# cudagu/aero-gnn

Hardware: AMD Instinct MI355X
Metric: million edge-updates/sec, 1M-node/6M-edge mesh, 1->8 MI355X (higher is better)
Workload: dtype bf16; 1 GPU; BSMS-MGN 4-scale U-Net train step (fwd+MSE+bwd+allreduce+Adam), 1000000 nodes / 5996000 edges per GPU; model=BiStridedMeshGraphNet(H=128, n_hid=2, processor_size=15, stride=2, concat_trick), mode=train, global_batch=1, parallelism=dp1

## Files before the change

### aero-gnn_amd/aerognn/_lib.py

```python
from __future__ import annotations

import ctypes as C
import os

_HERE = os.path.dirname(os.path.abspath(__file__))
LIB_PATH = os.environ.get("AEROGNN_LIB") or os.path.join(_HERE, "libaerognn.so")

MAX_LIN = 8
MAX_SEG = 3
F32, BF16, F16, F64 = 0, 1, 2, 3
SEG_PLAIN, SEG_GATHER, SEG_SUM, SEG_MEAN = 0, 1, 2, 3
OPT_RESIDENT = 0

vp = C.c_void_p
i32 = C.c_int


class Seg(C.Structure):
    _fields_ = [("kind", i32), ("k", i32), ("ld", i32), ("_pad", i32),
                ("ptr", vp), ("index", vp), ("store", vp)]


ACT = {"relu": 0, "gelu": 1, "silu": 2, "tanh": 3}

# ... 44 lines not shown
                ("w_in", vp), ("w_out", vp), ("out", vp), ("dout", vp), ("gw", vp), ("s_csc", vp), ("dh", vp),
                ("dpa", vp), ("dpb", vp), ("dtx", vp), ("dw_in", vp), ("partial", vp)]


class EdgeBwdArgs(C.Structure):
    _fields_ = [("rows", i32), ("nblk", i32), ("wpk", vp * 4), ("bias", vp * 4), ("ln_g", vp), ("e", vp),
                ("proj", vp), ("src", vp), ("dst", vp), ("g", vp), ("g2", vp), ("de", vp), ("g0", vp),
                ("dw_partial", vp), ("db_partial", vp), ("ln_partial", vp), ("stamps", vp),
                ("a1", vp), ("stats", vp), ("scratch", vp), ("wtpk0", vp),
                ("xk", i32), ("xld", i32)]


class EdgeFwdArgs(C.Structure):
    _fields_ = [("rows", i32), ("nblk", i32), ("wpk", vp * 4), ("bias", vp * 4), ("ln_g", vp), ("ln_b", vp),
                ("e", vp), ("proj", vp), ("src", vp), ("dst", vp), ("out", vp), ("act", vp * 3), ("hpre", vp),
                ("stats", vp)]


class PackDesc(C.Structure):
    _fields_ = [("src", vp), ("dst", vp), ("src_dtype", i32), ("dst_dtype", i32),
                ("rows", i32), ("cols", i32), ("trans", i32), ("ld", i32),
                ("row_off", i32), ("col_off", i32), ("dst_rows", i32), ("dst_cols", i32)]


class F64Seg(C.Structure):
    _fields_ = [("a", vp), ("aidx", vp), ("lda", i32), ("k", i32), ("w", vp), ("ldw", i32), ("transw", i32)]


class F64GemmArgs(C.Structure):
    _fields_ = [("rows", i32), ("n", i32), ("nseg", i32), ("_pad", i32), ("seg", F64Seg * 3), ("bias", vp),
                ("add", vp * 2), ("add_idx", vp * 2), ("add_ld", i32 * 2), ("mask", vp), ("mask_ld", i32),
# ... 5 lines not shown
    _fields_ = [("rows", i32), ("m", i32), ("k", i32), ("_pad", i32), ("g", vp), ("ldg", i32), ("_pad1", i32),
                ("x", vp), ("ldx", i32), ("_pad2", i32), ("xidx", vp), ("dw", vp), ("ldw", i32), ("_pad3", i32),
                ("db", vp)]


_lib = None

LAUNCHES = ("agn_pack", "agn_mlp_forward", "agn_mlp_backward", "agn_reduce_partials", "agn_wgrad", "agn_wgrad_segsum", "agn_colsum",
            "agn_segment_sum", "agn_segment_sum2", "agn_gather_rows", "agn_radix_sort_u64", "agn_row_ptr", "agn_row_ptr_i64",
            "agn_iota_keys", "agn_level_index",
            "agn_exclusive_scan_i32", "agn_pool_sort_keys", "agn_pool_assign", "agn_pool_edge_candidates",
            "agn_pool_edge_sort", "agn_pool_edge_emit", "agn_bfs_distance", "agn_center_seed", "agn_maxdeg_seed",
            "agn_bistride_select", "agn_index_map", "agn_subgraph_edges", "agn_scatter_rows", "agn_wec_forward",
            "agn_wec_backward", "agn_edge_features", "agn_node_features", "agn_normalize", "agn_col_stats", "agn_collate",
            "agn_segment_max", "agn_segment_max_backward", "agn_edge_bwd_fused", "agn_encoder_bwd_fused", "agn_wgrad_reduce",
            "agn_edge_forward32",
            "agn_proj_forward", "agn_proj_backward", "agn_fourier_embed", "agn_fourier_embed_bwd")


class AeroGNNError(RuntimeError):
    pass


class _Lib:

    def __init__(self, cdll):
        self._cdll = cdll
        for name in LAUNCHES:
            if hasattr(cdll, name):
                setattr(self, name, _timed_launch(getattr(cdll, name), name[4:]))

# ... 71 lines not shown
            "agn_index_map": (i32, [vp, i32, i32, vp, vp]),
            "agn_subgraph_edges": (i32, [vp, vp, i32, vp, vp, vp, C.POINTER(i32), vp, vp]),
            "agn_scatter_rows": (i32, [i32, i32, i32, vp, vp, i32, vp, i32, vp]),
            "agn_wec_blocks": (i32, [i32]),
            "agn_edge_bwd_blocks": (i32, [i32]),
            "agn_edge_bwd_scratch_bytes": (C.c_size_t, [i32]),
            "agn_edge_features": (i32, [i32, C.c_int64, i32, vp, vp, i32, vp, vp, vp, vp, vp]),
            "agn_normalize": (i32, [i32, i32, vp, i32, vp, vp, vp, i32, i32, vp]),
            "agn_col_stats_temp_bytes": (C.c_size_t, [i32, i32]),
            "agn_col_stats": (i32, [i32, i32, vp, i32, vp, vp, C.c_float, vp, vp]),
            "agn_collate": (i32, [i32, C.c_int64, C.c_int64, vp, vp, vp, vp, vp]),
            "agn_edge_bwd_fused": (i32, [C.POINTER(EdgeBwdArgs), vp]),
            "agn_encoder_bwd_fused": (i32, [C.POINTER(EdgeBwdArgs), vp]),
            "agn_edge_fwd32_blocks": (i32, [i32]),
            "agn_edge_forward32": (i32, [C.POINTER(EdgeFwdArgs), vp]),
            "agn_debug_node32_launches": (C.c_long, []),
            "agn_debug_enc32_launches": (C.c_long, []),
            "agn_debug_dec32_launches": (C.c_long, []),
            "agn_debug_node32_bwd_launches": (C.c_long, []),
            "agn_debug_dec32_bwd_launches": (C.c_long, []),
            "agn_fault_status": (i32, [C.POINTER(i32), i32]),
            "agn_fault_status_async": (i32, [vp, vp]),
            "agn_debug_set_fault": (i32, [i32]),
            "agn_wgrad_reduce": (i32, [C.POINTER(WgradBatch), i32, vp]),
            "agn_proj_forward": (i32, [i32, vp, i32, vp, vp, vp, i32, vp]),
            "agn_proj_backward": (i32, [i32, vp, vp, i32, vp, vp, i32, vp]),
            "agn_wec_forward": (i32, [C.POINTER(WecArgs), vp]),
            "agn_wec_backward": (i32, [C.POINTER(WecArgs), vp]),
            "agn_fourier_embed": (i32, [i32, i32, i32, vp, i32, i32, i32, i32, i32, vp, i32, vp]),
            "agn_fourier_embed_bwd": (i32, [i32, i32, i32, vp, i32, i32, i32, i32, i32, vp, i32, vp, i32, vp]),
# ... 39 lines not shown
```

### aero-gnn_amd/aerognn/core.py

```python
from __future__ import annotations

import ctypes as C

import torch

from . import _lib as L
from ._lib import check, ptr


def stream():
    return C.c_void_p(torch.cuda.current_stream().cuda_stream)


PROF = None
_TIMED_DEPTH = 0


class _Timed:
    __slots__ = ("tag", "cost", "s", "on")

    def __init__(self, tag, cost):
        self.tag, self.cost = tag, cost
        self.on = False

# ... 253 lines not shown
    return (os.environ.get("AEROGNN_FUSED_EDGE_BWD", "1") != "0" and dtype == torch.bfloat16 and hidden == 128
            and nlin == 4 and has_ln and rows >= 64 * 1024)


def edge32_ok(dtype, hidden, nlin, has_ln, act=0):
    import os
    return (os.environ.get("AEROGNN_EDGE32", "1") != "0" and dtype == torch.bfloat16 and hidden == 128
            and nlin == 4 and has_ln and act == 0)


def edge_saves_ok():
    import os
    return os.environ.get("AEROGNN_EB_SAVED", "1") != "0"


def edge_forward(*, rows, wpk, bias, ln, e, proj, src, dst, out, a1=None, stats=None, tag=None, cost=None):
    lib = L.lib()
    a = L.EdgeFwdArgs()
    a.rows = int(rows)
    a.nblk = int(lib.agn_edge_fwd32_blocks(int(rows)))
    for i in range(4):
        a.wpk[i] = wpk[i]
        a.bias[i] = bias[i]
    a.ln_g, a.ln_b = ln
    a.e, a.proj, a.src, a.dst, a.out = ptr(e), ptr(proj), ptr(src), ptr(dst), ptr(out)
    a.act[0] = ptr(a1)
    a.stats = ptr(stats)
    with timed(tag, cost):
        check(lib.agn_edge_forward32(C.byref(a), stream()), "edge_forward32")


FAULT_POLL_EVERY = 16
_fault = {"buf": None, "event": None, "n": 0, "dirty": False, "hooked": False, "word": 0}


def _fault_read(block, defer=False):
    st = _fault
    ev = st["event"]
    if ev is not None and (block or ev.query()):
        if block:
            ev.synchronize()
        st["word"] |= int(st["buf"][0])
        st["event"] = None
    f = st["word"]
# ... 282 lines not shown
                         None, 0, 0, 0, 0, None)
    scratch = None
    if rows > 0:
        check(lib.agn_wgrad_plan(C.byref(b)), "wgrad_plan")
        scratch = torch.empty(int(lib.agn_wgrad_partial_floats(128, 128, b.d[0].nsplit)), dtype=torch.float32,
                              device=G.device)
        b.d[0].dw_partial = ptr(scratch)
    s_el = G.element_size()
    io = rows * 256 * s_el + 4 * 128 * 129 + N * 128 * s_el + 4 * (N + 1)
    with timed(tag, (0.0, 2.0 * rows * 128 * 128, io)):
        check(lib.agn_wgrad_segsum(C.byref(b), dt_code(G.dtype), 0, ptr(rowptr), ptr(dst), N, ptr(out), out.stride(0), stream()),
              "wgrad_segsum")
    return out


def alg8d_edge(E, N, H, s, bwd=False):
    return (2 if bwd else 1) * (E * (2 * s * H + 8) + N * 2 * s * H)


def alg8d_node(N, H, s, bwd=False, proj=False):
    return (2 if bwd else 1) * N * 3 * s * H * (2 if (bwd and proj) else 1)


def with_alg(alg, impl):
    return (alg, impl[1], impl[0])


def mask_bytes(H):
    return 8 * max(1, (H + 63) // 64)


def cost_edge_fwd(E, N, H, s, nlin, train, a1_saves=False):
    per = 2 * H * s + 8 + ((nlin - 1) * (H * s + mask_bytes(H)) + H * s + 8 if train else 0)
    per += (H * s + 8) if a1_saves else 0
    return E * per + N * 2 * H * s, 2 * E * H * H * nlin


def cost_node_fwd(E, N, H, s, nlin, train):
    per = 2 * H * s + 8 + ((nlin - 1) * (H * s + mask_bytes(H)) + 2 * H * s + 8 if train else 0)
    return N * per + E * H * s, 2 * N * H * (2 * H + (nlin - 1) * H)


def cost_proj(N, H, s):
    return N * 3 * H * s, 2 * N * H * 2 * H


def cost_edge_bwd(E, N, H, s, nlin):
    per = H * s + H * s + (nlin - 1) * mask_bytes(H) + H * s + 8 + nlin * H * s + H * s + 4
    return E * per + N * H * s, 2 * E * H * H * nlin


def cost_edge_fwd_cat(E, N, H, s, nlin, train):
    per = 4 * H * s + 8 + ((nlin - 1) * (H * s + mask_bytes(H)) + H * s + 8 if train else 0)
    return E * per, 2 * E * H * (3 * H + (nlin - 1) * H)
# ... 30 lines not shown
```

### aero-gnn_amd/aerognn/functions.py

```python
from __future__ import annotations

import ctypes as C

import torch

from . import _lib as L
from ._lib import check, ptr
from . import core as _core
from .core import (Pack, WGrad, alg8d_edge, alg8d_node, with_alg, edge_bwd_fused, fused_edge_train_ok, bwd_nblocks,
                   edge32_ok, edge_saves_ok, edge_forward,
                   cost_edge_bwd_fused,
                   proj_kernel_ok, proj_forward, proj_backward, wgrad_dpd_ok, wgrad_segsum, tiled_empty, relu_mask_empty, colsum_rows, cost_edge_bwd, cost_edge_bwd_cat, cost_edge_fwd,
                   cost_edge_fwd_cat, cost_node_bwd, cost_node_fwd, cost_proj, cost_wec_bwd, cost_wec_fwd, dt_code,
                   timed, gather_rows, mlp_backward, mlp_forward, require_device,
                   scatter_rows, segment_max, segment_max_backward, segment_sum, segment_sum2, stream)


def _c(t):
    return t if t.is_contiguous() else t.contiguous()


def _ln_grads(partial, nblk, M, dtype):
    out = torch.empty(2 * M, dtype=torch.float32, device=partial.device)
    colsum_rows(partial, nblk, 2 * M, out)
    return out[:M].to(dtype), out[M:].to(dtype)
# ... 371 lines not shown
class GMPFn(torch.autograd.Function):

    @staticmethod
    def forward(ctx, x, e, level, spec: LayerSpec, train, *params):
        require_device(x, e)
        x, e = _c(x), _c(e)
        dt, dev = x.dtype, x.device
        N, E, H = x.shape[0], e.shape[0], spec.H
        es, ns = spec.edge, spec.node
        e_out = torch.empty_like(e)
        x_out = torch.empty_like(x)
        fused = train and spec.trick and fused_edge_train_ok(E, dt, H, es.nlin, es.ln is not None)
        e32 = (spec.trick and (fused or not train) and edge32_ok(dt, H, es.nlin, es.ln is not None, es.act)
               and e.stride(0) == H)
        saved = fused and e32 and edge_saves_ok()
        a1s = tiled_empty(E, H, dt, dev) if saved else None
        sts = torch.empty(E, 2, dtype=torch.float32, device=dev) if saved else None
        ea, ehp, est = _alloc_saves(es, E, dt, dev, train and not fused)
        na, nhp, nst = _alloc_saves(ns, N, dt, dev, train)
        P = None
        if spec.trick:
            P = torch.empty(N, 2 * H, dtype=dt, device=dev)
            sz = x.element_size()
            if proj_kernel_ok(x, H):
                proj_forward(N, x, spec.pack["proj"], spec.pack["proj_b"], P,
                             tag="proj", cost=with_alg(alg8d_node(N, H, sz), cost_proj(N, H, sz)))
            else:
                mlp_forward(rows=N, dtype=dt, hidden=H, nlin=1, out_dim=2 * H,
                            segs=[(L.SEG_PLAIN, x.shape[1], x.stride(0), x, None, None)],
                            wpk=[spec.pack["proj"]], bias=[spec.pack["proj_b"]], out=P,
                            tag="proj", cost=with_alg(alg8d_node(N, H, sz), cost_proj(N, H, sz)))
            if e32:
                edge_forward(rows=E, wpk=es.wpk(), bias=es.biases(), ln=es.lnp(), e=e, proj=P, src=level.src,
                             dst=level.dst, out=e_out, a1=a1s, stats=sts,
                             tag="edge_fwd", cost=with_alg(alg8d_edge(E, N, H, sz), cost_edge_fwd(E, N, H, sz, es.nlin,
                                                                                                 False, a1_saves=saved)))
            else:
                mlp_forward(rows=E, dtype=dt, hidden=H, nlin=es.nlin, act_fn=es.act, out_dim=H,
                            segs=[(L.SEG_PLAIN, H, e.stride(0), e, None, None)],
                            wpk=es.wpk(), bias=es.biases(), ln=es.lnp(), proj=P, src=level.src, dst=level.dst,
                            resid=e, out=e_out, acts=ea, hpre=ehp, stats=est,
                            tag="edge_fwd", cost=with_alg(alg8d_edge(E, N, H, sz), cost_edge_fwd(E, N, H, sz, es.nlin,
                                                                                                train and not fused)))
        else:
            se = (L.SEG_PLAIN, H, e.stride(0), e, None, None)
            ss = (L.SEG_GATHER, H, x.stride(0), x, level.src, None)
            sd = (L.SEG_GATHER, H, x.stride(0), x, level.dst, None)
            mlp_forward(rows=E, dtype=dt, hidden=H, nlin=es.nlin, act_fn=es.act, out_dim=H,
                        segs=[ss, sd, se] if spec.gmp_order else [se, ss, sd],
                        wpk=es.wpk(), bias=es.biases(), ln=es.lnp(), resid=e, out=e_out,
                        acts=ea, hpre=ehp, stats=est,
                        tag="edge_fwd", cost=with_alg(alg8d_edge(E, N, H, x.element_size()),
                                                       cost_edge_fwd_cat(E, N, H, x.element_size(), es.nlin, train)))
        kind = L.SEG_MEAN if spec.aggregation == "mean" else L.SEG_SUM
        agg = torch.empty(N, H, dtype=dt, device=dev) if train else None
        aseg = (kind, H, e_out.stride(0), e_out, level.rowptr, agg)
        mlp_forward(rows=N, dtype=dt, hidden=H, nlin=ns.nlin, act_fn=ns.act, out_dim=H,
                    segs=[(L.SEG_PLAIN, H, x.stride(0), x, None, None), aseg],
                    wpk=ns.wpk(), bias=ns.biases(), ln=ns.lnp(), resid=x, out=x_out,
                    acts=na, hpre=nhp, stats=nst,
                    tag="node_fwd", cost=with_alg(alg8d_node(N, H, x.element_size()),
                                                   cost_node_fwd(E, N, H, x.element_size(),
                                                                 ns.nlin, train)))
        ctx.spec, ctx.level = spec, level
        ctx.saves = (ea, ehp, est, na, nhp, nst, agg)
        ctx.fused, ctx.proj, ctx.esaves = fused, (P if fused and not saved else None), (a1s, sts)
        ctx.save_for_backward(x, e)
        ctx.set_materialize_grads(False)
        return x_out, e_out

    @staticmethod
    def backward(ctx, gx, ge):
        x, e = ctx.saved_tensors
        spec, lv = ctx.spec, ctx.level
        ea, ehp, est, na, nhp, nst, agg = ctx.saves
        es, ns = spec.edge, spec.node
        dt, dev = x.dtype, x.device
        N, E, H = x.shape[0], e.shape[0], spec.H
# ... 589 lines not shown
```

### aero-gnn_amd/csrc/edge32_fwd.hip

```cpp
#include "tile32.hpp"
#include "aerognn.h"

using namespace agn;
using namespace agn::t32;

namespace {

constexpr int LAYER = LAYER_UNITS;
#ifndef AGN_E32_PF
#define AGN_E32_PF 2
#endif
constexpr int PF = AGN_E32_PF;
#ifndef AGN_E32_DIAG
#define AGN_E32_DIAG 0
#endif

constexpr int NW = 12;

struct Smem {
  uint4 w[4 * LAYER];
  float pv[5][H];
  int ids[NW][64];
};
static_assert(sizeof(Smem) <= 160 * 1024, "LDS budget");

AGN_DEV void gemm4(f32x16 (&acc)[NT], const BOp<bf16, NR>& b, const uint4* w, int lane) {
  gemm_stream<PF>(acc, b, w, NU, 0, 0, lane);
}

#ifdef AGN_E32_STAMPS
__device__ unsigned long long* agn_e32_stamps;
#define E32_STAMP(k)                                                                                   \
  do {                                                                                                 \
    if (agn_e32_stamps && blockIdx.x == 0 && lane0 == 0 && ntile < 16)                                 \
      agn_e32_stamps[((threadIdx.x >> 6) * 16 + ntile) * 16 + (k)] =                                    \
          (k) == 15 ? __builtin_amdgcn_s_memrealtime() : __builtin_amdgcn_s_memtime();                   \
  } while (0)
#else
#define E32_STAMP(k) \
  do {               \
  } while (0)
#endif

template <bool SAVE>
__global__ __launch_bounds__(64 * NW) void edge32_fwd_kernel(const agn_edge_fwd_args a) {
  constexpr int NTHR = 64 * NW;
  __shared__ Smem sm;
  {
    const uint4* const* wp = reinterpret_cast<const uint4* const*>(a.wpk);
    for (int i = threadIdx.x; i < 4 * LAYER; i += NTHR) sm.w[i] = wp[i / LAYER][i % LAYER];
    for (int i = threadIdx.x; i < 5 * H; i += NTHR) {
      const int l = i / H, f = i - l * H;
      sm.pv[l][f] = l < 3 ? (a.bias[l + 1] ? a.bias[l + 1][f] : 0.f) : (l == 3 ? a.ln_g[f] : a.ln_b[f]);
    }
  }
  __syncthreads();
  const int lane0 = threadIdx.x & 63;
  const int w = __builtin_amdgcn_readfirstlane(threadIdx.x >> 6);
  const int ntiles = (a.rows + 31) / 32;
  const Walk walk(ntiles, w, NW);
  int* wids = sm.ids[w];
  const int32_t* const idp = lane0 < 32 ? a.src : a.dst;
  auto tile_id = [&](int t) { return idp[min(t * 32 + (lane0 & 31), a.rows - 1)]; };
  if (walk.first < walk.end) wids[lane0] = tile_id(walk.first);
  const bf16* P = reinterpret_cast<const bf16*>(a.proj);
  const bf16* E = reinterpret_cast<const bf16*>(a.e);
#ifdef AGN_E32_STAMPS
  int ntile = 0;
#endif
  for (int tile = walk.first; tile < walk.end; tile += walk.step) {
    cbarrier();
    E32_STAMP(0);
    E32_STAMP(15);
    const int lane = opaque_v(lane0);
    const int c = lane & 31, h = lane >> 5;
    const int row = tile * 32 + c;
    const bool valid = row < a.rows;
    const int rr = valid ? row : a.rows - 1;
    const bool more = tile + walk.step < walk.end;
    const int nid = tile_id(more ? tile + walk.step : tile);
    f32x16 acc[NT];
    BOp<bf16, NR> b;
    {
      const int cs = wids[c], cd = wids[32 + c];
      if (more) wids[lane] = nid;
      uint4 rs[NR / 8], rd[NR / 8];
      const bf16* ps = P + (size_t)cs * (2 * H) + 8 * h;
      const bf16* pd = P + (size_t)cd * (2 * H) + H + 8 * h;
#pragma unroll
      for (int i = 0; i < NR / 8; ++i) {
        rs[i] = *reinterpret_cast<const uint4*>(ps + 16 * i);
        rd[i] = *reinterpret_cast<const uint4*>(pd + 16 * i);
      }
      b.load_w(E + (size_t)rr * H, h);
      __builtin_amdgcn_sched_barrier(0);
      bf16x8 f0, f1;
      ident_frags_rows(f0, f1, lane);
      if (AGN_E32_DIAG == 3) {
#pragma unroll
// ... 37 lines not shown
      float v[NR];
#pragma unroll
      for (int i = 0; i < NR / 8; ++i) {
        float v8[8];
        acc_get8(v8, acc, i);
        ln_out8(v8, sm.pv[3], sm.pv[4], i, h, mean, rstd);
#pragma unroll
        for (int e = 0; e < 8; ++e) v[8 * i + e] = v8[e];
      }
      BOp<bf16, NR> lnb;
      lnb.set(v);
      bf16x8 f0, f1;
      ident_frags(f0, f1, lane);
      acc_add2_mfma<NT, NR>(acc, lnb, e0, f0, f1);
    }
#pragma unroll
    for (int i = 0; i < NR / 8; ++i) {
      float v[8];
      acc_get8(v, acc, i);
      store8_w(op, i, h, v, valid);
    }

    E32_STAMP(7);
#ifdef AGN_E32_STAMPS
    ++ntile;
#endif
  }
}

}

extern "C" {

#ifdef AGN_E32_STAMPS
int agn_debug_e32_stamps(void* p) {
  return hipMemcpyToSymbol(HIP_SYMBOL(agn_e32_stamps), &p, sizeof(p)) == hipSuccess ? 0 : -1;
}
#endif

int agn_edge_fwd32_blocks(int rows) {
  return tile_blocks((rows + 31) / 32, NW);
}

int agn_edge_forward32(const agn_edge_fwd_args* a, void* stream) {
  if (!a || a->rows < 0 || a->nblk < 1) return AGN_E_ARG;
  if (a->rows == 0) return 0;
  if (!a->e || !a->proj || !a->src || !a->dst || !a->out || !a->ln_g || !a->ln_b) return AGN_E_ARG;
  if (a->act[1] || a->act[2] || a->hpre) return AGN_E_ARG;
  const bool save = a->act[0] != nullptr;
  if (save != (a->stats != nullptr) || (save && (!al16(a->act[0]) || (reinterpret_cast<uintptr_t>(a->stats) & 7))))
    return AGN_E_ARG;
  for (int l = 0; l < 4; ++l)
    if (!a->wpk[l] || !al16(a->wpk[l])) return AGN_E_ARG;
  if (!al16(a->e) || !al16(a->proj) || !al16(a->out)) return AGN_E_ARG;
  if (save) hipLaunchKernelGGL(edge32_fwd_kernel<true>, dim3(a->nblk), dim3(64 * NW), 0, (hipStream_t)stream, *a);
  else hipLaunchKernelGGL(edge32_fwd_kernel<false>, dim3(a->nblk), dim3(64 * NW), 0, (hipStream_t)stream, *a);
  return launch_status();
}

}
```

### aero-gnn_amd/csrc/node32_fwd.hip

```cpp
#include "tile32.hpp"
#include "aerognn.h"

using namespace agn;
using namespace agn::t32;

namespace {

constexpr int L0 = 2 * LAYER_UNITS;
constexpr int L1 = LAYER_UNITS;
#ifndef AGN_N32_NW
#define AGN_N32_NW 8
#endif
#ifndef AGN_N32_NQ
#define AGN_N32_NQ 4
#endif
constexpr int NW = AGN_N32_NW;
constexpr int NQ = AGN_N32_NQ;
constexpr int PF = 2;

constexpr int PFG = 4;

template <int NLIN> struct Smem {
  uint4 w0[L0];
  uint4 w1[L1];
  uint4 w2[L1];
  float pv[NLIN + 2][H];
  int rp[NW][64];
  char agg[NW][2048];
};
static_assert(sizeof(Smem<4>) <= 160 * 1024, "LDS budget");


template <int NLIN, bool SAVES>
__global__ __launch_bounds__(64 * NW) void node32_fwd_kernel(const agn_mlp_fwd_args a) {
  constexpr int NTHR = 64 * NW;
  __shared__ Smem<NLIN> sm;
  {
    const uint4* w0 = reinterpret_cast<const uint4*>(a.wpk[0]);
    const uint4* w1 = reinterpret_cast<const uint4*>(a.wpk[1]);
    const uint4* w2 = reinterpret_cast<const uint4*>(a.wpk[2]);
    for (int i = threadIdx.x; i < L0; i += NTHR) sm.w0[i] = w0[i];
    for (int i = threadIdx.x; i < L1; i += NTHR) {
      sm.w1[i] = w1[i];
      sm.w2[i] = w2[i];
    }
    for (int i = threadIdx.x; i < (NLIN + 2) * H; i += NTHR) {
      const int l = i / H, f = i - l * H;
      const float* p = l < NLIN ? a.bias[l] : (l == NLIN ? a.ln_g : a.ln_b);
      sm.pv[l][f] = p ? p[f] : 0.f;
    }
  }
  __syncthreads();
  const int lane0 = threadIdx.x & 63;
  const int w = __builtin_amdgcn_readfirstlane(threadIdx.x >> 6);
  const int ntiles = (a.rows + 31) / 32;
  const Walk walk(ntiles, w, NW);
  int* wrp = sm.rp[w];
  const agn_seg& sx = a.seg[0];
  const agn_seg& sg = a.seg[1];
  const int32_t* const rowptr = sg.index;
  auto tile_rp = [&](int t) { return rowptr[min(t * 32 + min(lane0, 32), a.rows)]; };
  if (walk.first < walk.end) wrp[lane0] = tile_rp(walk.first);
  const bf16* X = reinterpret_cast<const bf16*>(sx.ptr);
  const bf16* EP = reinterpret_cast<const bf16*>(sg.ptr);
  for (int tile = walk.first; tile < walk.end; tile += walk.step) {
    cbarrier();
    const int lane = opaque_v(lane0);
    const int c = lane & 31, h = lane >> 5;
    const int row = tile * 32 + c;
    const bool valid = row < a.rows;
    const int rr = valid ? row : a.rows - 1;
    const bool more = tile + walk.step < walk.end;
    const int nrp = tile_rp(more ? tile + walk.step : tile);
    BOp<bf16, NR> bagg;
    {
      const int g = lane >> 4, k = lane & 15;
      char* buf = sm.agg[w];
      uint4 mine[NR / 8];
#pragma unroll
      for (int i = 0; i < NR / 8; ++i) mine[i] = uint4{0u, 0u, 0u, 0u};
      const bf16* ek = EP + 8 * k;
#pragma unroll 1
      for (int bt = 0; bt < 4; ++bt) {
        int beg[2], end[2];
#pragma unroll
        for (int n = 0; n < 2; ++n) {
          const int nl = 8 * bt + 4 * n + g;
          const int cc = tile * 32 + nl < a.rows ? nl : a.rows - 1 - tile * 32;
          beg[n] = wrp[cc];
          end[n] = wrp[cc + 1];
// ... 154 lines not shown

long g_launches = 0;

}

extern "C" long agn_debug_node32_launches(void) { return g_launches; }

namespace agn {
bool node32_fwd_try(const agn_mlp_fwd_args* a, void* stream, int* rc) {
  if (a->dtype != AGN_BF16 || a->hidden != H || (a->nlin != 3 && a->nlin != 4) || a->nseg != 2 || a->out_dim != H || !a->use_ln ||
      a->act_fn != AGN_ACT_RELU || a->proj || a->rows < 64 * 1024 || a->rows >= (1 << 26))
    return false;
  const agn_seg& sx = a->seg[0];
  const agn_seg& sg = a->seg[1];
  if (sx.kind != AGN_SEG_PLAIN || sx.k != H || sx.ld % 8 || !sx.ptr) return false;
  if ((sg.kind != AGN_SEG_SUM && sg.kind != AGN_SEG_MEAN) || sg.k != H || sg.ld % 8 || !sg.ptr || !sg.index) return false;
  if (a->resid != sx.ptr || a->out_ld != sx.ld || a->out_ld % 8) return false;
  bool saves = a->hpre || a->stats;
  for (int l = 0; l < AGN_MAX_LIN; ++l) {
    if (a->pre[l] || (l >= a->nlin - 1 && (a->act[l] || a->mask[l]))) return false;
    saves = saves || a->act[l] || a->mask[l];
    if (!al16(a->act[l])) return false;
  }
  if (!al16(a->hpre)) return false;
  for (int l = 0; l < a->nlin; ++l)
    if (!a->wpk[l] || !al16(a->wpk[l])) return false;
  if (!al16(sx.ptr) || !al16(sg.ptr) || !al16(a->out) || !al16(sg.store)) return false;
  const dim3 g(tile_blocks((a->rows + 31) / 32, NW)), blk(64 * NW);
  hipStream_t st = (hipStream_t)stream;
  if (a->nlin == 4) {
    if (saves) hipLaunchKernelGGL((node32_fwd_kernel<4, true>), g, blk, 0, st, *a);
    else hipLaunchKernelGGL((node32_fwd_kernel<4, false>), g, blk, 0, st, *a);
  } else {
    if (saves) hipLaunchKernelGGL((node32_fwd_kernel<3, true>), g, blk, 0, st, *a);
    else hipLaunchKernelGGL((node32_fwd_kernel<3, false>), g, blk, 0, st, *a);
  }
  ++g_launches;
  *rc = launch_status();
  return true;
}
}
```

### aero-gnn_amd/csrc/tile32.hpp

```cpp
#pragma once
#include "common.hpp"
#include "host.hpp"

namespace agn {
namespace t32 {

constexpr int H = 128;
constexpr int NT = 4;
constexpr int NR = 64;
constexpr int NU = 8;
constexpr int LAYER_UNITS = NT * NU * 64;

struct Walk {
  int first, end, step;
  AGN_DEV Walk(int ntiles, int w, int nw) {
    if (gridDim.x >= 8 && (gridDim.x & 7) == 0) {
      const int g = blockIdx.x & 7, bi = blockIdx.x >> 3, nb = gridDim.x >> 3;
      const int per = (ntiles + 7) / 8;
      first = g * per + bi * nw + w;
      end = min(ntiles, (g + 1) * per);
      step = nb * nw;
    } else {
      first = blockIdx.x * nw + w;
      end = ntiles;
      step = gridDim.x * nw;
    }
  }
};

template <int PF, bool FENCE = false>
AGN_DEV void gemm_stream(f32x16 (&acc)[NT], const BOp<bf16, NR>& b, const uint4* w, int ku_total, int ot0, int u0,
                         int lane) {
  uint4 f[PF];
#pragma unroll
  for (int i = 0; i < PF; ++i) f[i] = w[((ot0 + i % NT) * ku_total + u0 + i / NT) * 64 + lane];
#pragma unroll
  for (int idx = 0; idx < NT * NU; ++idx) {
    const uint4 cur = f[idx % PF];
    const int nx = idx + PF;
    if (nx < NT * NU) f[idx % PF] = w[((ot0 + nx % NT) * ku_total + u0 + nx / NT) * 64 + lane];
    b.mfma(acc[idx % NT], cur, idx / NT);
// ... 37 lines not shown
```

### include/aerognn.h

```cpp
#ifndef AEROGNN_H
#define AEROGNN_H
#include <stddef.h>
#include <stdint.h>
#ifdef __cplusplus
extern "C" {
#endif

#define AGN_MAX_LIN 8
#define AGN_MAX_SEG 3

enum { AGN_F32 = 0, AGN_BF16 = 1, AGN_F16 = 2, AGN_F64 = 3 };
enum { AGN_SEG_PLAIN = 0, AGN_SEG_GATHER = 1, AGN_SEG_SUM = 2, AGN_SEG_MEAN = 3 };
enum { AGN_E_ARG = -1, AGN_E_DTYPE = -2, AGN_E_HIDDEN = -3, AGN_E_SHAPE = -4 };
enum { AGN_ACT_RELU = 0, AGN_ACT_GELU = 1, AGN_ACT_SILU = 2, AGN_ACT_TANH = 3 };

typedef struct {
  int kind;
  int k;
  int ld;
  int _pad;
  const void* ptr;
  const int32_t* index;
  void* store;
} agn_seg;
// ... 244 lines not shown
typedef struct {
  int rows;
  int nblk;
  const void* wpk[4];
  const float* bias[4];
  const float* ln_g;
  const float* ln_b;
  const void* e;
  const void* proj;
  const int32_t* src;
  const int32_t* dst;
  void* out;
  void* act[3];
  void* hpre;
  float* stats;
} agn_edge_fwd_args;
int agn_edge_fwd32_blocks(int rows);
int agn_edge_forward32(const agn_edge_fwd_args* a, void* stream);
int agn_wgrad_reduce(const agn_wgrad_batch* b, int nsplit, void* stream);

int agn_proj_forward(int rows, const void* x, int x_ld, const void* wpk, const float* bias, void* out, int out_ld,
                     void* stream);
int agn_proj_backward(int rows, const void* dps, const void* dpd, int dp_ld, const void* wtpk, void* dx, int dx_ld,
                      void* stream);

int agn_edge_features(int ne, int64_t e_total, int pdim, const int64_t* edge_index, const float* pos, int pos_ld,
                      const int64_t* perm, const float* mean, const float* std, float* out, void* stream);
int agn_normalize(int n, int k, const float* x, int ld, const float* mean, const float* std, float* out, int out_ld,
                  int inverse, void* stream);
size_t agn_col_stats_temp_bytes(int n, int k);
int agn_col_stats(int n, int k, const float* x, int ld, float* mean, float* std, float eps, void* scratch,
                  void* stream);
int agn_collate(int B, int64_t ne, int64_t nn, const int64_t* edge_off, const int64_t* node_off, int64_t* edge_index,
// ... 56 lines not shown
```

Baseline: 810.1 M edge-updates/s.

## Fuse dst-sorted segment-sum aggregation into edge forward kernel with boundary fixup

The edge MLP forward kernel now walks contiguous tile ranges per wave and, using the dst-sorted edge order, accumulates edge outputs into per-node sums in LDS as it goes. Each completed segment is written straight to an agg buffer, and nodes with no incoming edges are zero-filled. A small fixup kernel recomputes segments that cross wave ranges. The node MLP then reads agg as a plain input instead of re-gathering E×H edge outputs by rowptr. This removes a full re-read of edge outputs, at the cost of serialized scan logic in the edge kernel, range-based scheduling instead of strided, extra LDS, and one extra launch.

```diff
diff --git a/aero-gnn_amd/aerognn/_lib.py b/aero-gnn_amd/aerognn/_lib.py
--- a/aero-gnn_amd/aerognn/_lib.py
+++ b/aero-gnn_amd/aerognn/_lib.py
@@ -82,7 +82,7 @@
 class EdgeFwdArgs(C.Structure):
     _fields_ = [("rows", i32), ("nblk", i32), ("wpk", vp * 4), ("bias", vp * 4), ("ln_g", vp), ("ln_b", vp),
                 ("e", vp), ("proj", vp), ("src", vp), ("dst", vp), ("out", vp), ("act", vp * 3), ("hpre", vp),
-                ("stats", vp)]
+                ("stats", vp), ("agg", vp), ("rowptr", vp), ("nodes", i32), ("_pad", i32)]
 
 
 class PackDesc(C.Structure):
@@ -118,7 +118,7 @@
             "agn_bistride_select", "agn_index_map", "agn_subgraph_edges", "agn_scatter_rows", "agn_wec_forward",
             "agn_wec_backward", "agn_edge_features", "agn_node_features", "agn_normalize", "agn_col_stats", "agn_collate",
             "agn_segment_max", "agn_segment_max_backward", "agn_edge_bwd_fused", "agn_encoder_bwd_fused", "agn_wgrad_reduce",
-            "agn_edge_forward32",
+            "agn_edge_forward32", "agn_edge_agg_fixup",
             "agn_proj_forward", "agn_proj_backward", "agn_fourier_embed", "agn_fourier_embed_bwd")
 
 
@@ -220,6 +220,8 @@
             "agn_encoder_bwd_fused": (i32, [C.POINTER(EdgeBwdArgs), vp]),
             "agn_edge_fwd32_blocks": (i32, [i32]),
             "agn_edge_forward32": (i32, [C.POINTER(EdgeFwdArgs), vp]),
+            "agn_edge_agg_fixup": (i32, [C.POINTER(EdgeFwdArgs), vp]),
+            "agn_debug_edge_agg_launches": (C.c_long, []),
             "agn_debug_node32_launches": (C.c_long, []),
             "agn_debug_enc32_launches": (C.c_long, []),
             "agn_debug_dec32_launches": (C.c_long, []),
diff --git a/aero-gnn_amd/aerognn/core.py b/aero-gnn_amd/aerognn/core.py
--- a/aero-gnn_amd/aerognn/core.py
+++ b/aero-gnn_amd/aerognn/core.py
@@ -291,7 +291,13 @@
     return os.environ.get("AEROGNN_EB_SAVED", "1") != "0"
 
 
-def edge_forward(*, rows, wpk, bias, ln, e, proj, src, dst, out, a1=None, stats=None, tag=None, cost=None):
+def edge_agg_ok(N, aggregation):
+    import os
+    return os.environ.get("AEROGNN_EDGE_AGG", "1") != "0" and aggregation == "add" and N >= 64 * 1024
+
+
+def edge_forward(*, rows, wpk, bias, ln, e, proj, src, dst, out, a1=None, stats=None, agg=None, rowptr=None,
+                 tag=None, cost=None):
     lib = L.lib()
     a = L.EdgeFwdArgs()
     a.rows = int(rows)
@@ -303,8 +309,16 @@
     a.e, a.proj, a.src, a.dst, a.out = ptr(e), ptr(proj), ptr(src), ptr(dst), ptr(out)
     a.act[0] = ptr(a1)
     a.stats = ptr(stats)
+    if agg is not None:
+        assert agg.dtype == out.dtype and agg.is_contiguous() and agg.shape[1] == 128
+        assert rowptr.dtype == torch.int32 and rowptr.is_contiguous() and rowptr.numel() == agg.shape[0] + 1
+        a.agg, a.rowptr, a.nodes = ptr(agg), ptr(rowptr), int(agg.shape[0])
     with timed(tag, cost):
         check(lib.agn_edge_forward32(C.byref(a), stream()), "edge_forward32")
+    if agg is not None:
+        nw = 12 * a.nblk
+        with timed("agg_fixup", (0.0, 0.0, 4 * nw + 256 * out.element_size() * nw)):
+            check(lib.agn_edge_agg_fixup(C.byref(a), stream()), "edge_agg_fixup")
 
 
 FAULT_POLL_EVERY = 16
@@ -617,8 +631,8 @@
     return out
 
 
-def alg8d_edge(E, N, H, s, bwd=False):
-    return (2 if bwd else 1) * (E * (2 * s * H + 8) + N * 2 * s * H)
+def alg8d_edge(E, N, H, s, bwd=False, agg=False):
+    return (2 if bwd else 1) * (E * (2 * s * H + 8) + N * 2 * s * H) + (N * s * H if agg else 0)
 
 
 def alg8d_node(N, H, s, bwd=False, proj=False):
@@ -633,14 +647,16 @@
     return 8 * max(1, (H + 63) // 64)
 
 
-def cost_edge_fwd(E, N, H, s, nlin, train, a1_saves=False):
+def cost_edge_fwd(E, N, H, s, nlin, train, a1_saves=False, agg=False):
     per = 2 * H * s + 8 + ((nlin - 1) * (H * s + mask_bytes(H)) + H * s + 8 if train else 0)
     per += (H * s + 8) if a1_saves else 0
-    return E * per + N * 2 * H * s, 2 * E * H * H * nlin
-
-
-def cost_node_fwd(E, N, H, s, nlin, train):
+    return E * per + N * 2 * H * s + (N * H * s if agg else 0), 2 * E * H * H * nlin
+
+
+def cost_node_fwd(E, N, H, s, nlin, train, plain_agg=False):
     per = 2 * H * s + 8 + ((nlin - 1) * (H * s + mask_bytes(H)) + 2 * H * s + 8 if train else 0)
+    if plain_agg:
+        return N * (per + H * s - (H * s if train else 0)), 2 * N * H * (2 * H + (nlin - 1) * H)
     return N * per + E * H * s, 2 * N * H * (2 * H + (nlin - 1) * H)
 
 
diff --git a/aero-gnn_amd/aerognn/functions.py b/aero-gnn_amd/aerognn/functions.py
--- a/aero-gnn_amd/aerognn/functions.py
+++ b/aero-gnn_amd/aerognn/functions.py
@@ -8,7 +8,7 @@
 from ._lib import check, ptr
 from . import core as _core
 from .core import (Pack, WGrad, alg8d_edge, alg8d_node, with_alg, edge_bwd_fused, fused_edge_train_ok, bwd_nblocks,
-                   edge32_ok, edge_saves_ok, edge_forward,
+                   edge32_ok, edge_saves_ok, edge_agg_ok, edge_forward,
                    cost_edge_bwd_fused,
                    proj_kernel_ok, proj_forward, proj_backward, wgrad_dpd_ok, wgrad_segsum, tiled_empty, relu_mask_empty, colsum_rows, cost_edge_bwd, cost_edge_bwd_cat, cost_edge_fwd,
                    cost_edge_fwd_cat, cost_node_bwd, cost_node_fwd, cost_proj, cost_wec_bwd, cost_wec_fwd, dt_code,
@@ -410,6 +410,8 @@
         e32 = (spec.trick and (fused or not train) and edge32_ok(dt, H, es.nlin, es.ln is not None, es.act)
                and e.stride(0) == H)
         saved = fused and e32 and edge_saves_ok()
+        eagg = e32 and edge_agg_ok(N, spec.aggregation)
+        agg = torch.empty(N, H, dtype=dt, device=dev) if eagg else None
         a1s = tiled_empty(E, H, dt, dev) if saved else None
         sts = torch.empty(E, 2, dtype=torch.float32, device=dev) if saved else None
         ea, ehp, est = _alloc_saves(es, E, dt, dev, train and not fused)
@@ -428,9 +430,10 @@
                             tag="proj", cost=with_alg(alg8d_node(N, H, sz), cost_proj(N, H, sz)))
             if e32:
                 edge_forward(rows=E, wpk=es.wpk(), bias=es.biases(), ln=es.lnp(), e=e, proj=P, src=level.src,
-                             dst=level.dst, out=e_out, a1=a1s, stats=sts,
-                             tag="edge_fwd", cost=with_alg(alg8d_edge(E, N, H, sz), cost_edge_fwd(E, N, H, sz, es.nlin,
-                                                                                                 False, a1_saves=saved)))
+                             dst=level.dst, out=e_out, a1=a1s, stats=sts, agg=agg, rowptr=level.rowptr if eagg else None,
+                             tag="edge_fwd", cost=with_alg(alg8d_edge(E, N, H, sz, agg=eagg),
+                                                           cost_edge_fwd(E, N, H, sz, es.nlin, False, a1_saves=saved,
+                                                                         agg=eagg)))
             else:
                 mlp_forward(rows=E, dtype=dt, hidden=H, nlin=es.nlin, act_fn=es.act, out_dim=H,
                             segs=[(L.SEG_PLAIN, H, e.stride(0), e, None, None)],
@@ -449,15 +452,18 @@
                         tag="edge_fwd", cost=with_alg(alg8d_edge(E, N, H, x.element_size()),
                                                        cost_edge_fwd_cat(E, N, H, x.element_size(), es.nlin, train)))
         kind = L.SEG_MEAN if spec.aggregation == "mean" else L.SEG_SUM
-        agg = torch.empty(N, H, dtype=dt, device=dev) if train else None
-        aseg = (kind, H, e_out.stride(0), e_out, level.rowptr, agg)
+        if eagg:
+            aseg = (L.SEG_PLAIN, H, agg.stride(0), agg, None, None)
+        else:
+            agg = torch.empty(N, H, dtype=dt, device=dev) if train else None
+            aseg = (kind, H, e_out.stride(0), e_out, level.rowptr, agg)
         mlp_forward(rows=N, dtype=dt, hidden=H, nlin=ns.nlin, act_fn=ns.act, out_dim=H,
                     segs=[(L.SEG_PLAIN, H, x.stride(0), x, None, None), aseg],
                     wpk=ns.wpk(), bias=ns.biases(), ln=ns.lnp(), resid=x, out=x_out,
                     acts=na, hpre=nhp, stats=nst,
                     tag="node_fwd", cost=with_alg(alg8d_node(N, H, x.element_size()),
                                                    cost_node_fwd(E, N, H, x.element_size(),
-                                                                 ns.nlin, train)))
+                                                                 ns.nlin, train, plain_agg=eagg)))
         ctx.spec, ctx.level = spec, level
         ctx.saves = (ea, ehp, est, na, nhp, nst, agg)
         ctx.fused, ctx.proj, ctx.esaves = fused, (P if fused and not saved else None), (a1s, sts)
diff --git a/aero-gnn_amd/csrc/edge32_fwd.hip b/aero-gnn_amd/csrc/edge32_fwd.hip
--- a/aero-gnn_amd/csrc/edge32_fwd.hip
+++ b/aero-gnn_amd/csrc/edge32_fwd.hip
@@ -1,3 +1,4 @@
+#include <type_traits>
 #include "tile32.hpp"
 #include "aerognn.h"
 
@@ -15,6 +16,9 @@
 #define AGN_E32_DIAG 0
 #endif
 
+#ifndef AGN_E32_AGG_DIAG
+#define AGN_E32_AGG_DIAG 0
+#endif
 constexpr int NW = 12;
 
 struct Smem {
@@ -23,6 +27,11 @@
   int ids[NW][64];
 };
 static_assert(sizeof(Smem) <= 160 * 1024, "LDS budget");
+struct SmemAgg : Smem {
+  uint4 stage[NW][8 * 16];
+};
+static_assert(sizeof(SmemAgg) <= 160 * 1024, "LDS budget");
+typedef const __attribute__((address_space(4))) int32_t* cidx_t;
 
 AGN_DEV void gemm4(f32x16 (&acc)[NT], const BOp<bf16, NR>& b, const uint4* w, int lane) {
   gemm_stream<PF>(acc, b, w, NU, 0, 0, lane);
@@ -42,10 +51,10 @@
   } while (0)
 #endif
 
-template <bool SAVE>
+template <bool SAVE, bool AGG>
 __global__ __launch_bounds__(64 * NW) void edge32_fwd_kernel(const agn_edge_fwd_args a) {
   constexpr int NTHR = 64 * NW;
-  __shared__ Smem sm;
+  __shared__ std::conditional_t<AGG, SmemAgg, Smem> sm;
   {
     const uint4* const* wp = reinterpret_cast<const uint4* const*>(a.wpk);
     for (int i = threadIdx.x; i < 4 * LAYER; i += NTHR) sm.w[i] = wp[i / LAYER][i % LAYER];
@@ -58,7 +67,7 @@
   const int lane0 = threadIdx.x & 63;
   const int w = __builtin_amdgcn_readfirstlane(threadIdx.x >> 6);
   const int ntiles = (a.rows + 31) / 32;
-  const Walk walk(ntiles, w, NW);
+  const std::conditional_t<AGG, RangeWalk, Walk> walk(ntiles, w, NW);
   int* wids = sm.ids[w];
   const int32_t* const idp = lane0 < 32 ? a.src : a.dst;
   auto tile_id = [&](int t) { return idp[min(t * 32 + (lane0 & 31), a.rows - 1)]; };
@@ -68,6 +77,20 @@
 #ifdef AGN_E32_STAMPS
   int ntile = 0;
 #endif
+  int cur = -1;
+  bool skip = true;
+  char* const aggp = reinterpret_cast<char*>(a.agg);
+  auto agg_put = [&](int n, uint32_t v, int l) {
+    if (AGN_E32_AGG_DIAG == 0 && (unsigned)n < (unsigned)a.nodes)
+      *reinterpret_cast<uint32_t*>(aggp + (size_t)n * (2 * H) + (uint32_t)(4 * l)) = v;
+  };
+  uint32_t* park = nullptr;
+  if constexpr (AGG && AGN_E32_AGG_DIAG != 1) {
+    park = reinterpret_cast<uint32_t*>(sm.stage[w]);
+    if (walk.first < walk.end && walk.first > 0) cur = ((cidx_t)(uintptr_t)a.dst)[walk.first * 32 - 1];
+    park[64 + lane0] = 0u;
+    park[128 + lane0] = 0u;
+  }
   for (int tile = walk.first; tile < walk.end; tile += walk.step) {
     cbarrier();
     E32_STAMP(0);
@@ -83,6 +106,7 @@
     BOp<bf16, NR> b;
     {
       const int cs = wids[c], cd = wids[32 + c];
+      if constexpr (AGG && AGN_E32_AGG_DIAG != 1) park[c] = cd;
       if (more) wids[lane] = nid;
       uint4 rs[NR / 8], rd[NR / 8];
       const bf16* ps = P + (size_t)cs * (2 * H) + 8 * h;
@@ -150,11 +174,64 @@
       ident_frags(f0, f1, lane);
       acc_add2_mfma<NT, NR>(acc, lnb, e0, f0, f1);
     }
-#pragma unroll
-    for (int i = 0; i < NR / 8; ++i) {
-      float v[8];
-      acc_get8(v, acc, i);
-      store8_w(op, i, h, v, valid);
+    if constexpr (!AGG || AGN_E32_AGG_DIAG == 1) {
+#pragma unroll
+      for (int i = 0; i < NR / 8; ++i) {
+        float v[8];
+        acc_get8(v, acc, i);
+        store8_w(op, i, h, v, valid);
+      }
+    } else {
+      u32x4 pk[NR / 8];
+#pragma unroll
+      for (int i = 0; i < NR / 8; ++i) {
+        float v[8];
+        acc_get8(v, acc, i);
+        pk[i] = __builtin_bit_cast(u32x4, pack8_w(v, h));
+        if (valid) *reinterpret_cast<u32x4*>(op + 16 * i + 8 * h) = pk[i];
+      }
+      char* const stg = reinterpret_cast<char*>(sm.stage[w]);
+      const int rcv = (int)park[c];
+      const int before = c > 0 ? (int)park[c - 1] : cur;
+      const int nrow = min(32, a.rows - tile * 32);
+      const uint32_t live = nrow >= 32 ? ~0u : (1u << nrow) - 1u;
+      const uint32_t brk = (uint32_t)__ballot(rcv != before) & live;
+      f32x2 s = {__uint_as_float(park[64 + lane]), __uint_as_float(park[128 + lane])};
+      const uint32_t wr = (uint32_t)(c & 7) * 256u, wx = (uint32_t)(c & 7) << 4;
+      const uint32_t rd = (uint32_t)lane << 2;
+#pragma unroll 1
+      for (int p = 0; p < 4; ++p) {
+        if ((c >> 3) == p) {
+#pragma unroll
+          for (int i = 0; i < NR / 8; ++i)
+            *reinterpret_cast<u32x4*>(stg + wr + (((uint32_t)(2 * i + h) << 4) ^ wx)) = pk[i];
+        }
+        uint32_t x[8];
+#pragma unroll
+        for (int r = 0; r < 8; ++r) x[r] = *reinterpret_cast<const uint32_t*>(stg + r * 256 + (rd ^ (uint32_t)(r << 4)));
+        const uint32_t bb = (brk >> (8 * p)) & 0xffu, lb = (live >> (8 * p)) & 0xffu;
+        if (bb == 0u && lb == 0xffu) {
+#pragma unroll
+          for (int r = 0; r < 8; ++r) s += f32x2{lo_bf16(x[r]), hi_bf16(x[r])};
+        } else {
+#pragma unroll
+          for (int r = 0; r < 8; ++r) {
+            if ((lb >> r) & 1u) {
+              if ((bb >> r) & 1u) {
+                const int d = __builtin_amdgcn_readlane(rcv, 8 * p + r);
+                if (!skip) agg_put(cur, pack2(s[0], s[1]), lane);
+                for (int n = cur + 1; n < d; ++n) agg_put(n, 0u, lane);
+                cur = d;
+                skip = false;
+                s = f32x2{0.f, 0.f};
+              }
+              s += f32x2{lo_bf16(x[r]), hi_bf16(x[r])};
+            }
+          }
+        }
+      }
+      park[64 + lane] = __float_as_uint(s[0]);
+      park[128 + lane] = __float_as_uint(s[1]);
     }
 
     E32_STAMP(7);
@@ -162,11 +239,57 @@
     ++ntile;
 #endif
   }
-}
+  if constexpr (AGG && AGN_E32_AGG_DIAG != 1) {
+    if (walk.first < walk.end) {
+      cbarrier();
+      const uint32_t sum = pack2(__uint_as_float(park[64 + lane0]), __uint_as_float(park[128 + lane0]));
+      const int rend = min(walk.end * 32, a.rows);
+      if (rend == a.rows) {
+        if (!skip) agg_put(cur, sum, lane0);
+        for (int n = cur + 1; n < a.nodes; ++n) agg_put(n, 0u, lane0);
+      } else if (!skip && ((cidx_t)(uintptr_t)a.dst)[rend] != cur) {
+        agg_put(cur, sum, lane0);
+      }
+    }
+  }
+}
+
+__global__ __launch_bounds__(256) void edge_agg_fixup_kernel(const agn_edge_fwd_args a) {
+  const int lane = threadIdx.x & 63;
+  const int gw = __builtin_amdgcn_readfirstlane(blockIdx.x * 4 + (threadIdx.x >> 6));
+  if (gw >= a.nblk * NW) return;
+  const int ntiles = (a.rows + 31) / 32;
+  const RangeWalk run(ntiles, a.nblk, gw / NW, gw % NW, NW);
+  if (run.first >= run.end || run.first == 0) return;
+  const cidx_t dst = (cidx_t)(uintptr_t)a.dst, ptr = (cidx_t)(uintptr_t)a.rowptr;
+  const int p = run.first * 32;
+  const int n = dst[p];
+  if (dst[p - 1] != n || (unsigned)n >= (unsigned)a.nodes) return;
+  const int beg = min(max(ptr[n], 0), a.rows), end = min(max(ptr[n + 1], beg), a.rows);
+  if (RangeWalk::first_of(ntiles, a.nblk, NW, run.first - 1) * 32 > beg) return;
+  const char* ep = reinterpret_cast<const char*>(a.out) + (uint32_t)(4 * lane);
+  float s0 = 0.f, s1 = 0.f;
+  for (int j = beg; j < end; j += 4) {
+    uint32_t v[4];
+#pragma unroll
+    for (int q = 0; q < 4; ++q) v[q] = *reinterpret_cast<const uint32_t*>(ep + (size_t)min(j + q, end - 1) * (2 * H));
+#pragma unroll
+    for (int q = 0; q < 4; ++q)
+      if (j + q < end) {
+        s0 += lo_bf16(v[q]);
+        s1 += hi_bf16(v[q]);
+      }
+  }
+  *reinterpret_cast<uint32_t*>(reinterpret_cast<char*>(a.agg) + (size_t)n * (2 * H) + (uint32_t)(4 * lane)) = pack2(s0, s1);
+}
+
+long g_agg_launches = 0;
 
 }
 
 extern "C" {
+
+long agn_debug_edge_agg_launches(void) { return g_agg_launches; }
 
 #ifdef AGN_E32_STAMPS
 int agn_debug_e32_stamps(void* p) {
@@ -180,7 +303,11 @@
 
 int agn_edge_forward32(const agn_edge_fwd_args* a, void* stream) {
   if (!a || a->rows < 0 || a->nblk < 1) return AGN_E_ARG;
-  if (a->rows == 0) return 0;
+  if (a->rows == 0) {
+    if (a->agg && a->nodes > 0 && hipMemsetAsync(a->agg, 0, (size_t)a->nodes * (2 * H), (hipStream_t)stream) != hipSuccess)
+      return launch_status();
+    return 0;
+  }
   if (!a->e || !a->proj || !a->src || !a->dst || !a->out || !a->ln_g || !a->ln_b) return AGN_E_ARG;
   if (a->act[1] || a->act[2] || a->hpre) return AGN_E_ARG;
   const bool save = a->act[0] != nullptr;
@@ -189,9 +316,27 @@
   for (int l = 0; l < 4; ++l)
     if (!a->wpk[l] || !al16(a->wpk[l])) return AGN_E_ARG;
   if (!al16(a->e) || !al16(a->proj) || !al16(a->out)) return AGN_E_ARG;
-  if (save) hipLaunchKernelGGL(edge32_fwd_kernel<true>, dim3(a->nblk), dim3(64 * NW), 0, (hipStream_t)stream, *a);
-  else hipLaunchKernelGGL(edge32_fwd_kernel<false>, dim3(a->nblk), dim3(64 * NW), 0, (hipStream_t)stream, *a);
+  if (a->agg && (!a->rowptr || a->nodes < 1 || !al16(a->agg))) return AGN_E_ARG;
+  const dim3 g(a->nblk), blk(64 * NW);
+  hipStream_t st = (hipStream_t)stream;
+  if (a->agg) {
+    ++g_agg_launches;
+    if (save) hipLaunchKernelGGL((edge32_fwd_kernel<true, true>), g, blk, 0, st, *a);
+    else hipLaunchKernelGGL((edge32_fwd_kernel<false, true>), g, blk, 0, st, *a);
+  } else {
+    if (save) hipLaunchKernelGGL((edge32_fwd_kernel<true, false>), g, blk, 0, st, *a);
+    else hipLaunchKernelGGL((edge32_fwd_kernel<false, false>), g, blk, 0, st, *a);
+  }
   return launch_status();
 }
 
-}
+int agn_edge_agg_fixup(const agn_edge_fwd_args* a, void* stream) {
+  if (!a || a->rows < 0 || a->nblk < 1 || a->nblk > (1 << 20)) return AGN_E_ARG;
+  if (!a->agg || !a->rowptr || a->nodes < 1 || !al16(a->agg)) return AGN_E_ARG;
+  if (a->rows == 0) return 0;
+  if (!a->dst || !a->out || !al16(a->out)) return AGN_E_ARG;
+  hipLaunchKernelGGL(edge_agg_fixup_kernel, dim3((a->nblk * NW + 3) / 4), dim3(256), 0, (hipStream_t)stream, *a);
+  return launch_status();
+}
+
+}
diff --git a/aero-gnn_amd/csrc/node32_fwd.hip b/aero-gnn_amd/csrc/node32_fwd.hip
--- a/aero-gnn_amd/csrc/node32_fwd.hip
+++ b/aero-gnn_amd/csrc/node32_fwd.hip
@@ -31,7 +31,7 @@
 static_assert(sizeof(Smem<4>) <= 160 * 1024, "LDS budget");
 
 
-template <int NLIN, bool SAVES>
+template <int NLIN, bool SAVES, bool PLAIN>
 __global__ __launch_bounds__(64 * NW) void node32_fwd_kernel(const agn_mlp_fwd_args a) {
   constexpr int NTHR = 64 * NW;
   __shared__ Smem<NLIN> sm;
@@ -60,7 +60,9 @@
   const agn_seg& sg = a.seg[1];
   const int32_t* const rowptr = sg.index;
   auto tile_rp = [&](int t) { return rowptr[min(t * 32 + min(lane0, 32), a.rows)]; };
-  if (walk.first < walk.end) wrp[lane0] = tile_rp(walk.first);
+  if constexpr (!PLAIN) {
+    if (walk.first < walk.end) wrp[lane0] = tile_rp(walk.first);
+  }
   const bf16* X = reinterpret_cast<const bf16*>(sx.ptr);
   const bf16* EP = reinterpret_cast<const bf16*>(sg.ptr);
   for (int tile = walk.first; tile < walk.end; tile += walk.step) {
@@ -71,9 +73,19 @@
     const bool valid = row < a.rows;
     const int rr = valid ? row : a.rows - 1;
     const bool more = tile + walk.step < walk.end;
-    const int nrp = tile_rp(more ? tile + walk.step : tile);
+    int nrp = 0;
+    if constexpr (!PLAIN) nrp = tile_rp(more ? tile + walk.step : tile);
     BOp<bf16, NR> bagg;
-    {
+    if constexpr (PLAIN) {
+      bagg.load_w(EP + (size_t)rr * sg.ld, h);
+#pragma unroll
+      for (int i = 0; i < NR / 8; ++i) {
+        u32x4 t = __builtin_bit_cast(u32x4, bagg.u[i]);
+        asm volatile("" : "+v"(t));
+        bagg.u[i] = __builtin_bit_cast(bf16x8, t);
+      }
+      __builtin_amdgcn_sched_barrier(0);
+    } else {
       const int g = lane >> 4, k = lane & 15;
       char* buf = sm.agg[w];
       uint4 mine[NR / 8];
@@ -258,7 +270,9 @@
   const agn_seg& sx = a->seg[0];
   const agn_seg& sg = a->seg[1];
   if (sx.kind != AGN_SEG_PLAIN || sx.k != H || sx.ld % 8 || !sx.ptr) return false;
-  if ((sg.kind != AGN_SEG_SUM && sg.kind != AGN_SEG_MEAN) || sg.k != H || sg.ld % 8 || !sg.ptr || !sg.index) return false;
+  const bool plain = sg.kind == AGN_SEG_PLAIN;
+  if ((!plain && sg.kind != AGN_SEG_SUM && sg.kind != AGN_SEG_MEAN) || sg.k != H || sg.ld % 8 || !sg.ptr) return false;
+  if (plain ? sg.store != nullptr : !sg.index) return false;
   if (a->resid != sx.ptr || a->out_ld != sx.ld || a->out_ld % 8) return false;
   bool saves = a->hpre || a->stats;
   for (int l = 0; l < AGN_MAX_LIN; ++l) {
@@ -272,12 +286,20 @@
   if (!al16(sx.ptr) || !al16(sg.ptr) || !al16(a->out) || !al16(sg.store)) return false;
   const dim3 g(tile_blocks((a->rows + 31) / 32, NW)), blk(64 * NW);
   hipStream_t st = (hipStream_t)stream;
-  if (a->nlin == 4) {
-    if (saves) hipLaunchKernelGGL((node32_fwd_kernel<4, true>), g, blk, 0, st, *a);
-    else hipLaunchKernelGGL((node32_fwd_kernel<4, false>), g, blk, 0, st, *a);
+  if (plain) {
+    if (a->nlin == 4) {
+      if (saves) hipLaunchKernelGGL((node32_fwd_kernel<4, true, true>), g, blk, 0, st, *a);
+      else hipLaunchKernelGGL((node32_fwd_kernel<4, false, true>), g, blk, 0, st, *a);
+    } else {
+      if (saves) hipLaunchKernelGGL((node32_fwd_kernel<3, true, true>), g, blk, 0, st, *a);
+      else hipLaunchKernelGGL((node32_fwd_kernel<3, false, true>), g, blk, 0, st, *a);
+    }
+  } else if (a->nlin == 4) {
+    if (saves) hipLaunchKernelGGL((node32_fwd_kernel<4, true, false>), g, blk, 0, st, *a);
+    else hipLaunchKernelGGL((node32_fwd_kernel<4, false, false>), g, blk, 0, st, *a);
   } else {
-    if (saves) hipLaunchKernelGGL((node32_fwd_kernel<3, true>), g, blk, 0, st, *a);
-    else hipLaunchKernelGGL((node32_fwd_kernel<3, false>), g, blk, 0, st, *a);
+    if (saves) hipLaunchKernelGGL((node32_fwd_kernel<3, true, false>), g, blk, 0, st, *a);
+    else hipLaunchKernelGGL((node32_fwd_kernel<3, false, false>), g, blk, 0, st, *a);
   }
   ++g_launches;
   *rc = launch_status();
diff --git a/aero-gnn_amd/csrc/tile32.hpp b/aero-gnn_amd/csrc/tile32.hpp
--- a/aero-gnn_amd/csrc/tile32.hpp
+++ b/aero-gnn_amd/csrc/tile32.hpp
@@ -25,6 +25,41 @@
       end = ntiles;
       step = gridDim.x * nw;
     }
+  }
+};
+
+struct RangeWalk {
+  int first, end, step;
+  static AGN_DEV void group(int ntiles, int grid, int blk, int w, int nw, int& base, int& cnt, int& i, int& n) {
+    if (grid >= 8 && (grid & 7) == 0) {
+      const int per = (ntiles + 7) / 8;
+      base = (blk & 7) * per;
+      cnt = max(0, min(ntiles, base + per) - base);
+      i = (blk >> 3) * nw + w;
+      n = (grid >> 3) * nw;
+    } else {
+      base = 0;
+      cnt = ntiles;
+      i = blk * nw + w;
+      n = grid * nw;
+    }
+  }
+  AGN_DEV RangeWalk(int ntiles, int grid, int blk, int w, int nw) {
+    int base, cnt, i, n;
+    group(ntiles, grid, blk, w, nw, base, cnt, i, n);
+    const int q = cnt / n, r = cnt - q * n;
+    first = base + i * q + min(i, r);
+    end = first + q + (i < r ? 1 : 0);
+    step = 1;
+  }
+  AGN_DEV RangeWalk(int ntiles, int w, int nw) : RangeWalk(ntiles, (int)gridDim.x, (int)blockIdx.x, w, nw) {}
+  static AGN_DEV int first_of(int ntiles, int grid, int nw, int t) {
+    int base, cnt, i, n;
+    const bool xcd = grid >= 8 && (grid & 7) == 0;
+    group(ntiles, grid, xcd ? t / ((ntiles + 7) / 8) : 0, 0, nw, base, cnt, i, n);
+    const int q = cnt / n, r = cnt - q * n, o = t - base;
+    const int k = o < r * (q + 1) ? o / (q + 1) : r + (o - r * (q + 1)) / q;
+    return base + k * q + min(k, r);
   }
 };
 
diff --git a/include/aerognn.h b/include/aerognn.h
--- a/include/aerognn.h
+++ b/include/aerognn.h
@@ -282,9 +282,15 @@
   void* act[3];
   void* hpre;
   float* stats;
+  void* agg;
+  const int32_t* rowptr;
+  int nodes;
+  int _pad;
 } agn_edge_fwd_args;
 int agn_edge_fwd32_blocks(int rows);
 int agn_edge_forward32(const agn_edge_fwd_args* a, void* stream);
+int agn_edge_agg_fixup(const agn_edge_fwd_args* a, void* stream);
+long agn_debug_edge_agg_launches(void);
 int agn_wgrad_reduce(const agn_wgrad_batch* b, int nsplit, void* stream);
 
 int agn_proj_forward(int rows, const void* x, int x_ld, const void* wpk, const float* bias, void* out, int out_ld,
```

New measurement: 825.7 M edge-updates/s, median of 6. 1.9% higher.
